# JanEGerken/HEAL-SWIN

Hardware: AMD Instinct MI355X
Metric: images/sec fwd+bwd, HEAL-SWIN nside=256 seg, batch=8 at 1/2/4/8 MI355X (higher is better)
Workload: dtype bf16

## Files before the change

heal_swin_amd/_lib.py:

```python
import ctypes
import os

import numpy as np

_PKG = os.path.dirname(os.path.abspath(__file__))
LIB_PATH = os.path.join(_PKG, "lib", "libhealswin.so")

HS_F32, HS_BF16 = 0, 1
HS_F64 = 3
HS_PRED_LABELS, HS_PRED_ROWS16 = 2, 4
HS_ENSEMBLE_PROB, HS_ENSEMBLE_LOGIT = 0, 1
HS_ATTN_COSINE = 1
HS_ATTN_FORCE_VALU = 2
HS_ATTN_RESIDUAL = 4
HS_ATTN_OVERWRITE_GRADS = 8
HS_EPI_BIAS, HS_EPI_GELU, HS_EPI_DGELU, HS_EPI_RESID = 0, 1, 2, 3
HS_ACC_DEFER = 2
HS_MLP_NORM_AFTER = 16
HS_U8, HS_I32, HS_I64 = 8, 9, 10
HS_FLAT_PATCH_ROWS, HS_FLAT_PIXEL_ROWS, HS_FLAT_IMAGE = 0, 1, 2
HS_DEPTH_L1, HS_DEPTH_L2, HS_DEPTH_HUBER, HS_DEPTH_LOGVAR = 0, 1, 2, 3
HS_DT_NONE, HS_DT_LOG, HS_DT_INV = 0, 1, 2
HS_DT_ZERO_BKG, HS_DT_1000_BKG, HS_DT_AFFINE, HS_DT_INVERSE = 1, 2, 4, 8
HS_DEPTH_STATS_WORDS = 15
# ... 157 lines not shown
    "hs_grad_scale": [c_ptr, c_i64, c_float, c_ptr, c_ptr],
    "hs_weight_avg_update": [c_ptr, c_ptr, c_i64, c_int, c_float, c_ptr, c_ptr, c_int, c_ptr],
    "hs_weight_avg_advance": [c_ptr, c_ptr, c_int, c_ptr],
    "hs_weight_avg_swap": [c_ptr, c_ptr, c_ptr, c_i64, c_ptr],
    "hs_split_bf16x3": [c_ptr, c_ptr, c_i64, c_int, c_int, c_ptr],
    "hs_gelu_split3": [c_ptr, c_ptr, c_ptr, c_i64, c_int, ctypes.c_float, ctypes.c_uint64, c_ptr],
    "hs_linear_wgrad_ld": [c_ptr, c_i64, c_i64, c_ptr, c_i64, c_i64, c_ptr, c_ptr, c_ptr, c_i64, c_int, c_int, c_int, c_ptr],
    "hs_layernorm_fwd": [c_ptr, c_ptr, c_ptr, c_ptr, c_ptr, c_ptr, c_ptr, c_i64, c_int, c_int, c_ptr],
    "hs_add_layernorm_fwd": [c_ptr, c_ptr, c_ptr, c_ptr, c_ptr, c_ptr, c_ptr, c_ptr, c_i64, c_int, c_int, c_ptr],
    "hs_add_layernorm_bwd": [c_ptr, c_ptr, c_ptr, c_ptr, c_ptr, c_ptr, c_ptr, c_ptr, c_ptr, c_ptr, c_int, c_i64, c_int, c_int, c_ptr],
    "hs_layernorm_drop_fwd": [c_ptr, c_ptr, c_ptr, c_ptr, c_ptr, c_ptr, c_ptr, c_ptr, c_i64, ctypes.c_float, ctypes.c_uint64,
                              c_i64, c_int, c_int, c_ptr],
    "hs_layernorm_drop_bwd": [c_ptr, c_ptr, c_ptr, c_ptr, c_ptr, c_ptr, c_ptr, c_ptr, c_ptr, c_int, c_ptr, c_i64, ctypes.c_float,
                              ctypes.c_uint64, c_i64, c_int, c_int, c_ptr],
    "hs_add_layernorm_drop_fwd": [c_ptr, c_ptr, c_ptr, c_ptr, c_ptr, c_ptr, c_ptr, c_ptr, c_ptr, c_i64, ctypes.c_float,
                                  ctypes.c_uint64, c_i64, c_int, c_int, c_ptr],
    "hs_layernorm_fwd_ex": [c_ptr, c_ptr, c_ptr, c_ptr, c_ptr, c_ptr, c_ptr, c_ptr, c_ptr, c_ptr, c_ptr, c_ptr, c_i64, ctypes.c_float,
                            ctypes.c_uint64, c_i64, c_int, c_int, c_ptr],
    "hs_add_layernorm_drop_bwd": [c_ptr, c_ptr, c_ptr, c_ptr, c_ptr, c_ptr, c_ptr, c_ptr, c_ptr, c_ptr, c_ptr, c_int, c_ptr, c_i64,
                                  ctypes.c_float, ctypes.c_uint64, c_i64, c_int, c_int, c_ptr],
    "hs_seg_ce_fwd": [c_ptr, c_ptr, c_ptr, c_ptr, c_i64, c_i64, c_int, c_i64, c_i64, c_i64, c_int, c_i64, c_int, c_ptr],
    "hs_seg_ce_bwd": [c_ptr, c_ptr, c_ptr, c_ptr, c_ptr, c_i64, c_i64, c_int, c_i64, c_i64, c_i64, c_i64, c_i64, c_i64, c_int, c_i64,
                      c_int, c_ptr],
    "hs_depth_loss_fwd": [c_ptr, c_ptr, c_ptr, c_i64, c_i64, c_int, c_i64, c_i64, c_i64, c_int, c_float, c_int, c_ptr],
    "hs_depth_loss_bwd": [c_ptr, c_ptr, c_ptr, c_ptr, c_i64, c_i64, c_int, c_i64, c_i64, c_i64, c_i64, c_i64, c_i64, c_int, c_float, c_int, c_ptr],
    "hs_gemm_nt": [c_ptr, c_i64, c_ptr, c_i64, c_int, c_ptr, c_i64, c_ptr, c_i64, c_int, c_ptr, c_ptr, c_ptr, c_i64, c_int, c_int,
                   ctypes.c_float, ctypes.c_uint64, c_int, c_ptr],
    "hs_lib_gemm_supported": [],
    "hs_lib_gemm_set_supported": [c_int],
    "hs_lib_gemm_nt": [c_ptr, c_ptr, c_ptr, c_int, c_ptr, c_ptr, c_i64, c_int, c_int, c_ptr],
    "hs_lib_gemm_pick": [c_i64, c_int, c_int, c_int, ctypes.POINTER(c_int), ctypes.POINTER(c_int), ctypes.c_char_p, c_int],
    "hs_lib_gemm_set_pick": [c_i64, c_int, c_int, c_int, c_int],
    "hs_gemm_nt_set_tile": [c_int],
    "hs_gemm_nt_tile_variant": [c_i64, c_int, c_int, c_int, c_int],
    "hs_set_reserved_cus": [c_int],
    "hs_transpose_many_16": [c_ptr, c_int, c_int, c_ptr],
    "hs_debug_occupy_cus": [c_int, c_int, c_int, ctypes.c_double, c_ptr],
    "hs_debug_buffer_soffset_probe": [c_ptr, c_int, c_int, c_ptr, c_ptr],
    "hs_window_attn_module_supported": [c_int, c_int, c_int, c_int],
    "hs_window_attn_module_fwd": [c_ptr, c_ptr, c_ptr, c_ptr, c_ptr, c_ptr, c_ptr, c_ptr, c_ptr, c_ptr, c_ptr, c_i64, c_ptr, c_int, c_i64,
                                  c_int, c_int, c_int, c_uint, c_int, c_ptr],
    "hs_window_attn_module_fwd_train": [c_ptr] * 17 + [c_i64] + [c_ptr] * 6 + [c_int, c_i64, c_int, c_int, c_int, c_uint, c_int, c_ptr],
    "hs_window_attn_module_bwd_chain": [c_ptr] * 14 + [c_i64] + [c_ptr] * 11 + [c_int, c_int, c_i64, c_int, c_int, c_int, c_uint, c_int, c_ptr],
    "hs_layernorm_bwd": [c_ptr, c_ptr, c_ptr, c_ptr, c_ptr, c_ptr, c_ptr, c_ptr, c_ptr, c_int, c_i64, c_int, c_int, c_ptr],
    "hs_patch_merge_fwd": [c_ptr, c_ptr, c_ptr, c_ptr, c_ptr, c_ptr, c_ptr, c_ptr, c_i64, c_int, c_int, c_int, c_ptr],
    "hs_patch_merge_bwd": [c_ptr, c_ptr, c_ptr, c_ptr, c_ptr, c_ptr, c_ptr, c_ptr, c_ptr, c_ptr, c_ptr, c_ptr, c_ptr, c_int, c_i64,
                           c_int, c_int, c_int, c_ptr],
    "hs_patch_expand_fwd": [c_ptr, c_ptr, c_ptr, c_ptr, c_ptr, c_ptr, c_ptr, c_ptr, c_i64, c_int, c_int, c_int, c_int, c_ptr],
    "hs_patch_expand_bwd": [c_ptr, c_ptr, c_ptr, c_ptr, c_ptr, c_ptr, c_ptr, c_ptr, c_ptr, c_ptr, c_ptr, c_ptr, c_ptr, c_int, c_i64,
                            c_int, c_int, c_int, c_int, c_ptr],
}
_OTHER = {
    "hs_version": ([], ctypes.c_char_p),
    "hs_last_error": ([], ctypes.c_char_p),
    "hs_status_string": ([c_int], ctypes.c_char_p),
    "hs_device_count": ([], c_int),
    "hs_get_reserved_cus": ([], c_int),
    "hs_grad_guard_piece": ([], c_int),
    "hs_adam_max_groups": ([], c_int),
    "hs_get_seed_epoch": ([], c_ptr),
    "hs_reduce_pending": ([c_ptr], c_int),
    "hs_layernorm_bwd_workspace": ([c_i64, c_int], c_i64),
    "hs_seg_ce_partials": ([c_i64, c_i64], c_i64),
    "hs_depth_loss_partials": ([c_i64, c_i64], c_i64),
    "hs_depth_points_workspace": ([c_i64, c_i64], c_i64),
    "hs_depth_metrics_partials": ([c_i64], c_i64),
# ... 163 lines not shown
```

heal_swin_amd/csrc/expand_ln_head.hip:

```cpp
#include "ln_head_device.h"
#include "hs_depth_loss.h"

#pragma clang fp contract(off)
#include "hs_depth_target.h"
#include "hs_depth_metrics.h"
#pragma clang fp contract(fast)

namespace hs {
namespace {

constexpr int kP = 4;
constexpr int kRowB = 256;
constexpr int kPatchRow = 128;

constexpr int kHistBins = kKP * kKP;

__device__ __forceinline__ int argmax_merge(float best, int arg, float ob, int oa) {
    const bool n0 = best != best, n1 = ob != ob;
    const int lower = arg < oa ? arg : oa;
    if (n0 || n1) return n0 && n1 ? lower : (n0 ? arg : oa);
    return best > ob ? arg : (ob > best ? oa : lower);
}

struct TailLane {
    float num = 0.f, den = 0.f;
    uint32_t pred4 = 0;
    uint32_t bad_rows = 0;
    uint32_t* hist = nullptr;
    float4 m4, lv4;
    double dsum[depth_metrics::kNSums];
};

struct TailCe {
    const uint8_t* labels;
    const float* class_w;
    float* loss_part;
    int n_classes;
    __device__ __forceinline__ bool has_loss() const { return labels != nullptr; }
    __device__ __forceinline__ bool ce_row(TailLane& st, const f32x16& lg, const float (&bk)[8], int64_t orow, bool live, int half,
                                           float (&v)[8], int& yl) const {
        if (!labels) return false;
        float m = -INFINITY;
#pragma unroll
        for (int r = 0; r < 8; ++r) {
            v[r] = lg[r] + bk[r];
            if (class_natural(r, half) < n_classes) m = fmaxf(m, v[r]);
        }
        m = fmaxf(m, __shfl_xor(m, 32, 64));
        yl = live ? (int)labels[orow] : 255;
        float ssum = 0.f, pick = 0.f;
#pragma unroll
        for (int r = 0; r < 8; ++r) {
            const int cls = class_natural(r, half);
            if (cls < n_classes) ssum += __builtin_amdgcn_exp2f((v[r] - m) * kLog2e);
            pick = cls == yl ? v[r] : pick;
        }
        ssum += __shfl_xor(ssum, 32, 64);
        pick += __shfl_xor(pick, 32, 64);
        const float wy = yl < n_classes ? (class_w ? class_w[yl] : 1.f) : 0.f;
        if (half == 0) {
            st.num = fmaf(wy, m + __builtin_amdgcn_logf(ssum) * kLn2 - pick, st.num);
            st.den += wy;
        }
        return true;
    }
    __device__ __forceinline__ void row(TailLane& st, const f32x16& lg, const float (&bk)[8], int64_t orow, int, bool live,
                                        int lane) const {
        float v[8];
        int yl;
        ce_row(st, lg, bk, orow, live, lane >> 5, v, yl);
    }
};

struct TailCeStep : TailCe {
    uint8_t* preds;
    unsigned long long* conf;
    unsigned long long* bad;
    __device__ __forceinline__ bool has_loss() const { return true; }
    __device__ __forceinline__ void row(TailLane& st, const f32x16& lg, const float (&bk)[8], int64_t orow, int p, bool live,
                                        int lane) const {
        const int half = lane >> 5;
        float v[8];
        int yl;
        if (!ce_row(st, lg, bk, orow, live, half, v, yl)) return;
        float best = -INFINITY;
        int arg = 4 * half < n_classes ? 4 * half : 64;
#pragma unroll
        for (int r = 0; r < 8; ++r) {
            const int cls = class_natural(r, half);
            if (cls < n_classes && !(best != best) && (v[r] > best || v[r] != v[r])) {
                best = v[r];
                arg = cls;
            }
        }
        const int pred = argmax_merge(best, arg, __shfl_xor(best, 32, 64), __shfl_xor(arg, 32, 64));
        st.pred4 |= (uint32_t)pred << (8 * p);
        if (conf) {
            const bool mine = live && half == 0;
            const int bin = mine && yl < n_classes ? yl * n_classes + pred : -1;
            st.bad_rows += (uint32_t)__popcll(__ballot(mine && yl >= n_classes));
            const int lead = __builtin_amdgcn_readfirstlane(bin);
            const unsigned long long same = __ballot(bin == lead);
            if (bin == lead) {
                if (lead >= 0 && lane == __ffsll((long long)same) - 1) atomicAdd(&st.hist[lead], (uint32_t)__popcll(same));
            } else if (bin >= 0) {
                atomicAdd(&st.hist[bin], 1u);
            }
        }
    }
};

struct TailDepth {
    const float* target;
    float* loss_part;
    int kind;
    float delta;
    __device__ __forceinline__ bool has_loss() const { return true; }
    __device__ __forceinline__ float depth_row(TailLane& st, const f32x16& lg, const float (&bk)[8], int64_t orow, bool live,
                                               int half) const {
        const float t = live && half == 0 ? target[orow] : INFINITY;
        if (depth_keep(t)) {
            st.num += depth_term(kind, delta, lg[0] + bk[0], lg[1] + bk[1], t);
            st.den += 1.f;
        }
        return t;
    }
    __device__ __forceinline__ void row(TailLane& st, const f32x16& lg, const float (&bk)[8], int64_t orow, int, bool live,
                                        int lane) const {
        depth_row(st, lg, bk, orow, live, lane >> 5);
    }
};

struct TailDepthStep : TailDepth {
    int n_out;
    TargetOp inv;
    depth_metrics::Rule rule;
    double* partial;
    float* preds;
    float* logvar_out;
    int64_t rows;
    __device__ __forceinline__ void row(TailLane& st, const f32x16& lg, const float (&bk)[8], int64_t orow, int p, bool live,
                                        int lane) const {
        const int half = lane >> 5;
        const float p0 = lg[0] + bk[0], p1 = lg[1] + bk[1], t = depth_row(st, lg, bk, orow, live, half);
        if (partial || preds) {
#pragma clang fp contract(off)
            const float m = target_op(p0, inv);
            if (partial && live && half == 0)
                depth_metrics::accumulate<float, float>(st.dsum, rule, m, target_op(t, inv), [&] { return p1; });
            st.m4.x = p == 0 ? m : st.m4.x;
            st.m4.y = p == 1 ? m : st.m4.y;
            st.m4.z = p == 2 ? m : st.m4.z;
            st.m4.w = p == 3 ? m : st.m4.w;
        }
        st.lv4.x = p == 0 ? p1 : st.lv4.x;
        st.lv4.y = p == 1 ? p1 : st.lv4.y;
        st.lv4.z = p == 2 ? p1 : st.lv4.z;
        st.lv4.w = p == 3 ? p1 : st.lv4.w;
    }
};

template <int NB, typename Loss>
__global__ void __launch_bounds__(256, 1) expand_ln_head_fwd_kernel(const uint16_t* __restrict__ xn, const uint16_t* __restrict__ xn_lo,
                                                                    const uint16_t* __restrict__ wexp,
                                                                    const uint16_t* __restrict__ wfold, const float* __restrict__ bvec,
                                                                    uint16_t* __restrict__ y, float* __restrict__ logits,
                                                                    float* __restrict__ mean_out, float* __restrict__ rstd_out,
                                                                    int64_t tokens, Loss ce) {
    constexpr bool kStep = std::is_same<Loss, TailCeStep>::value, kDStep = std::is_same<Loss, TailDepthStep>::value;
    constexpr int C = 32 * NB, KS = 2 * NB, NCH = C / 8;
    extern __shared__ __attribute__((aligned(16))) unsigned char smem[];
    unsigned char* wl = smem;
    unsigned char* patch = smem + kP * C * kRowB + (threadIdx.x >> 6) * (32 * kPatchRow);
    const int tid = threadIdx.x, lane = tid & 63, l31 = lane & 31, half = lane >> 5;

    for (int q = tid; q < kP * C * NCH; q += 256) {
        const int row = q / NCH, ch = q % NCH;
        *(uint4*)(wl + row * kRowB + ((ch ^ (row & 15)) << 4)) = *(const uint4*)(wexp + (int64_t)row * C + ch * 8);
    }
    bf16x8 wfa[NB][2], wfl[NB][2];
#pragma unroll
    for (int ct = 0; ct < NB; ++ct)
#pragma unroll
        for (int j = 0; j < 2; ++j) {
            const uint16_t* src = wfold + l31 * C + 32 * ct + 16 * j + 4 * half;
            const uint2 a = *(const uint2*)src, b = *(const uint2*)(src + 8);
            wfa[ct][j] = __builtin_bit_cast(bf16x8, make_uint4(a.x, a.y, b.x, b.y));
            const uint2 al = *(const uint2*)(src + 32 * C), bl = *(const uint2*)(src + 32 * C + 8);
            wfl[ct][j] = __builtin_bit_cast(bf16x8, make_uint4(al.x, al.y, bl.x, bl.y));
        }
    float bk[8];
    load_head_bias(bvec, half, bk);
    uint32_t* hist = (uint32_t*)(smem + kP * C * kRowB + 4 * 32 * kPatchRow);
    TailLane st;
    st.hist = hist + (tid >> 6) * kHistBins;
    if constexpr (kStep) {
        for (int j = tid; j < 4 * kHistBins; j += 256) hist[j] = 0;
    }
    if constexpr (kDStep) {
#pragma unroll
        for (int k = 0; k < depth_metrics::kNSums; ++k) st.dsum[k] = 0.0;
    }
    __syncthreads();

    const int sx = l31 & 15;
    const int64_t wave = (int64_t)blockIdx.x * 4 + (tid >> 6), nwaves = (int64_t)gridDim.x * 4;
    for (int64_t tok0 = wave * 32; tok0 < tokens; tok0 += nwaves * 32) {
        const int64_t tok = tok0 + l31;
        const bool live = tok < tokens;
        bf16x8 xb[KS];
#pragma unroll
        for (int ks = 0; ks < KS; ++ks) {
            const uint4 v = live ? *(const uint4*)(xn + tok * C + 16 * ks + 8 * half) : make_uint4(0, 0, 0, 0);
            xb[ks] = __builtin_bit_cast(bf16x8, v);
        }
        st.pred4 = 0;
        st.m4 = st.lv4 = make_float4(0.f, 0.f, 0.f, 0.f);
#pragma unroll 1
        for (int p = 0; p < kP; ++p) {
            f32x16 acc[NB];
#pragma unroll
            for (int ct = 0; ct < NB; ++ct)
#pragma unroll
                for (int r = 0; r < 16; ++r) acc[ct][r] = 0.f;
            const unsigned char* wrow = wl + (p * C + l31) * kRowB;
#pragma unroll
            for (int ks = 0; ks < KS; ++ks) {
                const int co = ((2 * ks + half) ^ sx) << 4;
#pragma unroll
                for (int ct = 0; ct < NB; ++ct) {
                    const bf16x8 a = *(const bf16x8*)(wrow + ct * 32 * kRowB + co);
                    acc[ct] = __builtin_amdgcn_mfma_f32_32x32x16_bf16(a, xb[ks], acc[ct], 0, 0, 0);
                }
            }
            if (xn_lo) {
#pragma unroll
                for (int ks = 0; ks < KS; ++ks) {
                    const uint4 v = live ? *(const uint4*)(xn_lo + tok * C + 16 * ks + 8 * half) : make_uint4(0, 0, 0, 0);
                    const int co = ((2 * ks + half) ^ sx) << 4;
#pragma unroll
                    for (int ct = 0; ct < NB; ++ct) {
                        const bf16x8 a = *(const bf16x8*)(wrow + ct * 32 * kRowB + co);
                        acc[ct] = __builtin_amdgcn_mfma_f32_32x32x16_bf16(a, __builtin_bit_cast(bf16x8, v), acc[ct], 0, 0, 0);
                    }
                }
            }
            const int64_t orow = tok * kP + p;
            if (y) {
#pragma unroll
                for (int pr = 0; pr < (NB + 1) / 2; ++pr) {
#pragma unroll
                    for (int t = 0; t < 2; ++t) {
                        const int ct = 2 * pr + t;
                        if (ct < NB) {
#pragma unroll
                            for (int g = 0; g < 4; ++g) {
                                const int chunk = 4 * t + g;
                                *(uint2*)(patch + l31 * kPatchRow + ((chunk ^ (l31 & 7)) << 4) + 8 * half) =
                                    make_uint2(pack_bf16x2(acc[ct][4 * g], acc[ct][4 * g + 1]), pack_bf16x2(acc[ct][4 * g + 2], acc[ct][4 * g + 3]));
                            }
                        }
                    }
                    __builtin_amdgcn_fence(__ATOMIC_RELEASE, "wavefront");
                    __builtin_amdgcn_wave_barrier();
                    constexpr int kChunksLast = (NB % 2) ? 4 : 8;
                    const int nchunks = (2 * pr + 1 < NB) ? 8 : kChunksLast;
#pragma unroll
                    for (int i = 0; i < 4; ++i) {
                        const int q = lane + 64 * i, row = q >> 3, chunk = q & 7;
                        const uint4 v = *(const uint4*)(patch + row * kPatchRow + ((chunk ^ (row & 7)) << 4));
                        if (chunk < nchunks && tok0 + row < tokens)
                            *(uint4*)(y + ((tok0 + row) * kP + p) * C + 64 * pr + chunk * 8) = v;
                    }
                    __builtin_amdgcn_fence(__ATOMIC_ACQUIRE, "wavefront");
                    __builtin_amdgcn_wave_barrier();
                }
            }
            float mean, rstd;
            row_stats<16>(acc, mean, rstd);
            f32x16 lg;
#pragma unroll
            for (int r = 0; r < 16; ++r) lg[r] = 0.f;
#pragma unroll
            for (int ct = 0; ct < NB; ++ct)
#pragma unroll
                for (int j = 0; j < 2; ++j) {
                    float xh[8];
#pragma unroll
                    for (int i = 0; i < 8; ++i) xh[i] = acc[ct][8 * j + i] * rstd;
                    lg = head_step<3>(lg, xh, wfa[ct][j], wfl[ct][j]);
                }
            ce.row(st, lg, bk, orow, p, live, lane);
            if (live) {
                if (logits) {
                    *(float4*)(logits + orow * kKP + 4 * half) = make_float4(lg[0] + bk[0], lg[1] + bk[1], lg[2] + bk[2], lg[3] + bk[3]);
                    *(float4*)(logits + orow * kKP + 8 + 4 * half) = make_float4(lg[4] + bk[4], lg[5] + bk[5], lg[6] + bk[6], lg[7] + bk[7]);
                }
                if (half == 0 && mean_out) {
                    mean_out[orow] = mean;
                    rstd_out[orow] = rstd;
                }
            }
        }
        if constexpr (kStep) {
            if (ce.preds && live && half == 0) *(uint32_t*)(ce.preds + tok * kP) = st.pred4;
        }
        if constexpr (kDStep) {
            if (live && half == 0) {
                if (ce.preds) *(float4*)(ce.preds + tok * kP) = st.m4;
                float* lv = ce.preds ? (ce.n_out > 1 ? ce.preds + ce.rows : nullptr) : ce.logvar_out;
                if (lv) *(float4*)(lv + tok * kP) = st.lv4;
            }
        }
    }
    if constexpr (kDStep) {
        if (ce.partial) {
            constexpr int NS = depth_metrics::kNSums;
            static_assert(NS * 256 * sizeof(double) <= kP * 64 * kRowB + 4 * 32 * kPatchRow, "lane sums must fit the LDS at C = 64");
            double* red = (double*)smem;
            __syncthreads();
#pragma unroll
            for (int k = 0; k < NS; ++k) red[k * 256 + tid] = st.dsum[k];
            __syncthreads();
            for (int h = 128; h > 0; h >>= 1) {
                for (int q = tid; q < NS * h; q += 256) {
                    const int k = q / h, j = q - k * h;
                    red[k * 256 + j] += red[k * 256 + j + h];
                }
                __syncthreads();
            }
            if (tid < NS) ce.partial[(int64_t)blockIdx.x * NS + tid] = red[tid * 256];
        }
    }
    if constexpr (kStep) {
        if (ce.conf) {
            __syncthreads();
            const int bins = ce.n_classes * ce.n_classes;
            if (tid < bins) {
                const uint32_t n = hist[tid] + hist[kHistBins + tid] + hist[2 * kHistBins + tid] + hist[3 * kHistBins + tid];
                if (n) atomicAdd(&ce.conf[tid], (unsigned long long)n);
            }
            if (lane == 0 && st.bad_rows) atomicAdd(&ce.bad[0], (unsigned long long)st.bad_rows);
        }
    }
    if (ce.has_loss()) {
        const float n = wave_sum(st.num), d = wave_sum(st.den);
        if (lane == 0) {
            ce.loss_part[2 * wave] = n;
            ce.loss_part[2 * wave + 1] = d;
        }
    }
}

}
}

extern "C" {

int hs_expand_ln_head_supported(int width, int children, int n_classes, int dtype) {
    return dtype == HS_BF16 && children == hs::kP && width % 32 == 0 && width >= 64 && width <= 128 && n_classes >= 1 && n_classes <= 16;
}

extern "C++" {
namespace {
template <typename Loss>
int launch_expand_ln_head(const void* xn, const void* xn_lo, const void* wexp, const void* wfold, const float* bvec, void* y, float* logits,
                          float* mean, float* rstd, int64_t tokens, int width, int children, int dtype, void* stream, Loss ce,
                          const char* who) {
    using namespace hs;
    HS_CHECK_ARG(xn && wexp && wfold && bvec, "%s: null pointer", who);
    HS_CHECK_ARG(tokens > 0, "%s: bad shape", who);
    HS_CHECK_ARG((y == nullptr) == (mean == nullptr) && (mean == nullptr) == (rstd == nullptr),
                 "%s: y, mean and rstd (what the backward needs) go together", who);
    if (!hs_expand_ln_head_supported(width, children, 1, dtype))
        return fail(HS_ERR_UNSUPPORTED, "%s: bf16, 4 children, C in {64, 96, 128} (got C = %d, children %d): the expand "
                    "weight must fit the LDS", who, width, children);
    HS_CHECK_ALIGNED(who, 16, xn, xn_lo, wexp, wfold, bvec, y);
    constexpr bool kStep = std::is_same<Loss, TailCeStep>::value;
    const size_t smem = (size_t)kP * width * kRowB + 4 * 32 * kPatchRow + (kStep ? 4 * kHistBins * sizeof(uint32_t) : 0);
    HS_CHECK_ARG(smem <= 160 * 1024, "%s: %zu bytes of LDS", who, smem);
    const dim3 grid((unsigned)hs_expand_ln_head_blocks(tokens)), block(256);
    if constexpr (kStep) {
        const int64_t groups = (tokens + 31) / 32, waves = (int64_t)grid.x * 4;
        HS_CHECK_ARG((groups + waves - 1) / waves < (1ll << 25), "%s: %lld tokens on %lld waves overflow the 32-bit histogram bins", who,
                     (long long)tokens, (long long)waves);
    }
    return with_width_blocks<4>(width, [&](auto nb) {
        auto kern = expand_ln_head_fwd_kernel<decltype(nb)::value, Loss>;
        static bool configured = false;
        if (!configured) {
            HS_HIP_CHECK(hipFuncSetAttribute((const void*)kern, hipFuncAttributeMaxDynamicSharedMemorySize, (int)smem));
            configured = true;
        }
        hipLaunchKernelGGL(kern, grid, block, smem, (hipStream_t)stream, (const uint16_t*)xn, (const uint16_t*)xn_lo,
                           (const uint16_t*)wexp, (const uint16_t*)wfold, bvec, (uint16_t*)y, logits, mean, rstd, tokens, ce);
        HS_LAUNCH_CHECK("expand_ln_head_fwd");
        return (int)HS_OK;
    });
}
int check_ce_loss(const char* who, const void* labels, const void* loss_partials, int n_classes) {
    HS_CHECK_ARG(labels && loss_partials, "%s: null pointer", who);
    return hs::check_class_count(who, n_classes);
}
int check_depth_loss(const char* who, const void* target, const void* loss_partials, int kind, float huber_delta, int n_out) {
    HS_CHECK_ARG(target && loss_partials, "%s: null pointer", who);
    return hs::check_depth_head(who, kind, huber_delta, n_out);
}
}
}

int64_t hs_expand_ln_head_blocks(int64_t tokens) {
    int64_t blocks = (tokens + 127) / 128;
    const int cus = hs::usable_cus();
    if (blocks > cus) blocks = cus;
    return blocks < 1 ? 1 : blocks;
}

int hs_expand_ln_head_fwd(const void* xn, const void* xn_lo, const void* wexp, const void* wfold, const float* bvec, void* y, float* logits,
                          float* mean, float* rstd, int64_t tokens, int width, int children, int dtype, void* stream) {
    HS_CHECK_ARG(logits, "hs_expand_ln_head_fwd: null pointer");
    return launch_expand_ln_head(xn, xn_lo, wexp, wfold, bvec, y, logits, mean, rstd, tokens, width, children, dtype, stream,
                                 hs::TailCe{nullptr, nullptr, nullptr, 0}, "hs_expand_ln_head_fwd");
}

int hs_expand_ln_head_ce_fwd(const void* xn, const void* xn_lo, const void* wexp, const void* wfold, const float* bvec, const uint8_t* labels,
                             const float* class_weights, int n_classes, void* y, float* logits, float* mean, float* rstd,
                             float* loss_partials, int64_t tokens, int width, int children, int dtype, void* stream) {
    if (int e = check_ce_loss("hs_expand_ln_head_ce_fwd", labels, loss_partials, n_classes)) return e;
    return launch_expand_ln_head(xn, xn_lo, wexp, wfold, bvec, y, logits, mean, rstd, tokens, width, children, dtype, stream,
                                 hs::TailCe{labels, class_weights, loss_partials, n_classes}, "hs_expand_ln_head_ce_fwd");
}

int hs_expand_ln_head_ce_step_fwd(const void* xn, const void* xn_lo, const void* wexp, const void* wfold, const float* bvec,
                                  const uint8_t* labels, const float* class_weights, int n_classes, void* y, float* logits, float* mean,
                                  float* rstd, float* loss_partials, uint8_t* preds, int64_t* confmat, int64_t* bad, int64_t tokens,
                                  int width, int children, int dtype, void* stream) {
    const char* who = "hs_expand_ln_head_ce_step_fwd";
    if (int e = check_ce_loss(who, labels, loss_partials, n_classes)) return e;
    HS_CHECK_ARG(!confmat || bad, "%s: confmat needs bad (the counter of labels >= n_classes)", who);
    HS_CHECK_ARG(((uintptr_t)preds & 3) == 0, "%s: preds must be 4-byte aligned", who);
    return launch_expand_ln_head(xn, xn_lo, wexp, wfold, bvec, y, logits, mean, rstd, tokens, width, children, dtype, stream,
                                 hs::TailCeStep{{labels, class_weights, loss_partials, n_classes}, preds, (unsigned long long*)confmat,
                                                (unsigned long long*)bad}, who);
}

int hs_expand_ln_head_depth_step_fwd(const void* xn, const void* xn_lo, const void* wexp, const void* wfold, const float* bvec,
                                     const float* target, int kind, float huber_delta, int n_out, void* y, float* logits, float* mean,
                                     float* rstd, float* loss_partials, int flags, int transform, float shift, float scale, int use_logvar,
                                     double total_mean, const float* ranges, int n_ranges, double* metric_partials, double* metric_state,
                                     float* preds, float* logvar_out, int64_t tokens, int width, int children, int dtype, void* stream) {
    const char* who = "hs_expand_ln_head_depth_step_fwd";
    if (int e = check_depth_loss(who, target, loss_partials, kind, huber_delta, n_out)) return e;
    HS_CHECK_ARG(transform == HS_DT_NONE || transform == HS_DT_LOG || transform == HS_DT_INV, "%s: transform %d", who, transform);
    HS_CHECK_ARG((flags & ~(HS_DT_AFFINE | HS_DT_INVERSE)) == 0, "%s: flags %d (HS_DT_AFFINE or 0: the inverse chain is applied)", who, flags);
    HS_CHECK_ARG((metric_partials == nullptr) == (metric_state == nullptr), "%s: metric_partials and metric_state go together", who);
    HS_CHECK_ARG(n_out == 2 || !(logvar_out || (use_logvar && metric_state)), "%s: the log variance needs a two-channel head", who);
    hs::TailDepthStep st{{target, loss_partials, kind, huber_delta}, n_out, hs::TargetOp{flags | HS_DT_INVERSE, transform, shift, scale},
                         {}, metric_partials, preds, logvar_out, tokens * hs::kP};
    if (int e = hs::depth_metrics::fill_rule(st.rule, use_logvar, total_mean, ranges, n_ranges)) return e;
    HS_CHECK_ALIGNED(who, 16, preds, logvar_out);
    HS_CHECK_ALIGNED(who, 8, metric_partials, metric_state);
    HS_CHECK_ALIGNED(who, 4, target, loss_partials);
    if (int e = launch_expand_ln_head(xn, xn_lo, wexp, wfold, bvec, y, logits, mean, rstd, tokens, width, children, dtype, stream, st, who))
        return e;
    if (metric_state) {
        hipLaunchKernelGGL(hs::depth_metrics::reduce_kernel, dim3(1), dim3(hs::depth_metrics::kThreads), 0, (hipStream_t)stream,
                           metric_partials, (int)hs_expand_ln_head_blocks(tokens), metric_state);
        HS_LAUNCH_CHECK("expand_ln_head_depth_step_reduce");
    }
    return HS_OK;
}

int hs_expand_ln_head_depth_fwd(const void* xn, const void* xn_lo, const void* wexp, const void* wfold, const float* bvec, const float* target,
                                int kind, float huber_delta, int n_out, void* y, float* logits, float* mean, float* rstd, float* loss_partials,
                                int64_t tokens, int width, int children, int dtype, void* stream) {
    if (int e = check_depth_loss("hs_expand_ln_head_depth_fwd", target, loss_partials, kind, huber_delta, n_out)) return e;
    return launch_expand_ln_head(xn, xn_lo, wexp, wfold, bvec, y, logits, mean, rstd, tokens, width, children, dtype, stream,
                                 hs::TailDepth{target, loss_partials, kind, huber_delta}, "hs_expand_ln_head_depth_fwd");
}

}
```

include/healswin.h:

```cpp
#ifndef HEALSWIN_H
#define HEALSWIN_H

#include <stdint.h>

#ifdef __cplusplus
extern "C" {
#endif

typedef enum {
    HS_OK = 0,
    HS_ERR_INVALID_ARG = 1,
    HS_ERR_UNSUPPORTED = 2,
    HS_ERR_HIP = 3,
    HS_ERR_NOT_PERMUTATION = 4,
    HS_ERR_MISALIGNED = 5
} hs_status;

typedef enum { HS_F32 = 0, HS_BF16 = 1 } hs_dtype;

#define HS_ATTN_COSINE 1u
#define HS_ATTN_FORCE_VALU 2u
#define HS_ATTN_RESIDUAL 4u
#define HS_ATTN_OVERWRITE_GRADS 8u

// ... 364 lines not shown
int hs_sample_bilinear_u8_f32_per_sample(const void* img, int batch, int channels, int height, int width, const double* rx,
                                         const double* ry, int64_t n, float* out, void* stream);
int hs_sample_nearest_f32_per_sample(const float* src, int batch, int height, int width, const double* rx, const double* ry, int64_t n,
                                     float background, float* out, void* stream);
int hs_depth_target(const float* in, int64_t in_stride_b, int64_t in_stride_p, float* out, int64_t out_stride_b, int64_t out_stride_p,
                    int64_t batch, int64_t n, int flags, int transform, float shift, float scale, void* stream);
int64_t hs_depth_stats_partials(int64_t n);
int hs_depth_stats_update(const float* depth, int64_t n, int transform, int use_masking, int64_t* partial, int64_t* state, void* stream);
int hs_depth_stats_merge(const int64_t* states, int count, int64_t* state, void* stream);
int hs_histogram_update(const float* depth, int64_t n, int transform, int use_masking, const double* edges, int bins, int64_t* counts,
                        void* stream);

int64_t hs_select_rows_workspace(int rows);
int hs_select_rows(const float* x, int rows, int64_t n, int64_t row_stride, int64_t k, int nan_propagates, int splits, void* workspace,
                   float* out, void* stream);

int hs_ln_head_supported(int width, int n_classes, int dtype);
int64_t hs_ln_head_partials(int64_t rows);
int hs_ln_head_fwd(const void* y, const void* wfold, const float* bvec, void* logits, float* mean, float* rstd, int64_t rows,
                   int width, int dtype, int logits_dtype, void* stream);
int hs_ln_head_bwd(const void* y, const float* mean, const float* rstd, const void* dlogits, const void* afold, void* dy,
                   void* dprime, float* partials, int64_t rows, int width, int dtype, int logits_dtype, void* stream);

int hs_split_bf16x3(const float* x, void* out, int64_t rows, int k, int mode, void* stream);
int hs_gelu_split3(const float* dy, const float* x, void* out3, int64_t rows, int k, float drop_p, uint64_t seed, void* stream);
int hs_linear_wgrad_ld(const void* dy, int64_t ldy, int64_t ycol0, const void* x, int64_t ldx, int64_t xcol0, float* dw, float* dbias,
                       float* workspace, int64_t rows, int n_out, int k_in, int accumulate, void* stream);

int hs_expand_ln_head_supported(int width, int children, int n_classes, int dtype);
int hs_expand_ln_head_fwd(const void* xn, const void* xn_lo, const void* wexp, const void* wfold, const float* bvec, void* y, float* logits,
                          float* mean, float* rstd, int64_t tokens, int width, int children, int dtype, void* stream);

int64_t hs_expand_ln_head_blocks(int64_t tokens);
int hs_expand_ln_head_ce_fwd(const void* xn, const void* xn_lo, const void* wexp, const void* wfold, const float* bvec, const uint8_t* labels,
                             const float* class_weights, int n_classes, void* y, float* logits, float* mean, float* rstd,
                             float* loss_partials, int64_t tokens, int width, int children, int dtype, void* stream);
int hs_expand_ln_head_ce_step_fwd(const void* xn, const void* xn_lo, const void* wexp, const void* wfold, const float* bvec,
                                  const uint8_t* labels, const float* class_weights, int n_classes, void* y, float* logits, float* mean,
                                  float* rstd, float* loss_partials, uint8_t* preds, int64_t* confmat, int64_t* bad, int64_t tokens,
                                  int width, int children, int dtype, void* stream);
int hs_ln_head_ce_bwd(const void* y, const float* mean, const float* rstd, const uint8_t* labels, const float* class_weights,
                      const float* scale, int n_classes, const void* wfold, const float* bvec, const void* afold, void* dy, void* dprime,
                      float* partials, int64_t rows, int width, int dtype, void* stream);

int hs_expand_ln_head_depth_fwd(const void* xn, const void* xn_lo, const void* wexp, const void* wfold, const float* bvec, const float* target,
                                int kind, float huber_delta, int n_out, void* y, float* logits, float* mean, float* rstd, float* loss_partials,
                                int64_t tokens, int width, int children, int dtype, void* stream);
int hs_expand_ln_head_depth_step_fwd(const void* xn, const void* xn_lo, const void* wexp, const void* wfold, const float* bvec,
                                     const float* target, int kind, float huber_delta, int n_out, void* y, float* logits, float* mean,
                                     float* rstd, float* loss_partials, int flags, int transform, float shift, float scale, int use_logvar,
                                     double total_mean, const float* ranges, int n_ranges, double* metric_partials, double* metric_state,
                                     float* preds, float* logvar_out, int64_t tokens, int width, int children, int dtype, void* stream);
int hs_ln_head_depth_bwd(const void* y, const float* mean, const float* rstd, const float* target, int kind, float huber_delta,
                         const float* scale, int n_out, const void* wfold, const float* bvec, const void* afold, void* dy, void* dprime,
                         float* partials, int64_t rows, int width, int dtype, void* stream);

int hs_patch_merge_fwd(const void* x, const float* gamma, const float* beta, const void* w, void* normed, float* mean, float* rstd,
                       void* out, int64_t rows, int dim, int dim_out, int dtype, void* stream);
int64_t hs_patch_merge_bwd_workspace(int64_t rows, int dim, int dim_out);
int hs_patch_merge_bwd(const void* dout, const void* x, const void* normed, const float* gamma, const float* mean, const float* rstd,
                       const void* w_t, void* dnormed, void* dx, float* dw, float* dgamma, float* dbeta, float* workspace,
                       int accumulate, int64_t rows, int dim, int dim_out, int dtype, void* stream);
int hs_patch_expand_fwd(const void* x, const void* w, const float* gamma, const float* beta, void* expanded, float* mean, float* rstd,
                        void* out, int64_t rows, int dim, int dim_exp, int children, int dtype, void* stream);
int64_t hs_patch_expand_bwd_workspace(int64_t rows, int dim, int dim_exp, int children);
int hs_patch_expand_bwd(const void* dout, const void* x, const void* expanded, const float* gamma, const float* mean, const float* rstd,
// ... 30 lines not shown
```

Measured before the change: 57.23.

## Run expand-LN-head tail kernel with 8 waves per block and lean register use

Adds an 8-wave-per-workgroup variant of the fused expand+layernorm+head kernel, the default for CE losses. To fit registers it reloads the input per child instead of holding it across the loop, shrinks the patch staging buffer for the step variant, and prefetches four labels per token with class weights shuffled across lanes instead of loaded per row. Loss partials from the extra waves are folded through LDS so the partial-buffer layout stays 4 slots per block, and unused slots are zeroed. The aim is more latency hiding per CU, paid for with extra global reloads and tighter LDS use.

```diff
diff --git a/heal_swin_amd/_lib.py b/heal_swin_amd/_lib.py
--- a/heal_swin_amd/_lib.py
+++ b/heal_swin_amd/_lib.py
@@ -213,6 +213,9 @@
     "hs_lib_gemm_pick": [c_i64, c_int, c_int, c_int, ctypes.POINTER(c_int), ctypes.POINTER(c_int), ctypes.c_char_p, c_int],
     "hs_lib_gemm_set_pick": [c_i64, c_int, c_int, c_int, c_int],
     "hs_gemm_nt_set_tile": [c_int],
+    "hs_expand_ln_head_set_waves": [c_int],
+    "hs_expand_ln_head_set_max_blocks": [c_int],
+    "hs_expand_ln_head_waves": [c_int],
     "hs_gemm_nt_tile_variant": [c_i64, c_int, c_int, c_int, c_int],
     "hs_set_reserved_cus": [c_int],
     "hs_transpose_many_16": [c_ptr, c_int, c_int, c_ptr],
diff --git a/heal_swin_amd/csrc/expand_ln_head.hip b/heal_swin_amd/csrc/expand_ln_head.hip
--- a/heal_swin_amd/csrc/expand_ln_head.hip
+++ b/heal_swin_amd/csrc/expand_ln_head.hip
@@ -27,6 +27,8 @@
     uint32_t pred4 = 0;
     uint32_t bad_rows = 0;
     uint32_t* hist = nullptr;
+    uint32_t lab4 = 0;
+    float cw = 1.f;
     float4 m4, lv4;
     double dsum[depth_metrics::kNSums];
 };
@@ -37,7 +39,19 @@
     float* loss_part;
     int n_classes;
     __device__ __forceinline__ bool has_loss() const { return labels != nullptr; }
-    __device__ __forceinline__ bool ce_row(TailLane& st, const f32x16& lg, const float (&bk)[8], int64_t orow, bool live, int half,
+    __device__ __forceinline__ void prepare(TailLane& st, int lane) const {
+        if (labels) st.cw = class_w ? ((lane & 15) < n_classes ? class_w[lane & 15] : 0.f) : 1.f;
+    }
+    __device__ __forceinline__ void fetch(TailLane& st, int64_t tok, bool live) const {
+        if (!labels) return;
+        const uint8_t* lp = labels + tok * 4;
+        if (((uintptr_t)labels & 3) == 0)
+            st.lab4 = live ? *(const uint32_t*)lp : 0xffffffffu;
+        else
+            st.lab4 = live ? (uint32_t)lp[0] | (uint32_t)lp[1] << 8 | (uint32_t)lp[2] << 16 | (uint32_t)lp[3] << 24 : 0xffffffffu;
+    }
+    template <bool PRE>
+    __device__ __forceinline__ bool ce_row(TailLane& st, const f32x16& lg, const float (&bk)[8], int64_t orow, int p, bool live, int half,
                                            float (&v)[8], int& yl) const {
         if (!labels) return false;
         float m = -INFINITY;
@@ -47,7 +61,7 @@
             if (class_natural(r, half) < n_classes) m = fmaxf(m, v[r]);
         }
         m = fmaxf(m, __shfl_xor(m, 32, 64));
-        yl = live ? (int)labels[orow] : 255;
+        yl = PRE ? (int)((st.lab4 >> (8 * p)) & 255u) : (live ? (int)labels[orow] : 255);
         float ssum = 0.f, pick = 0.f;
 #pragma unroll
         for (int r = 0; r < 8; ++r) {
@@ -57,18 +71,25 @@
         }
         ssum += __shfl_xor(ssum, 32, 64);
         pick += __shfl_xor(pick, 32, 64);
-        const float wy = yl < n_classes ? (class_w ? class_w[yl] : 1.f) : 0.f;
+        float wy;
+        if constexpr (PRE) {
+            const float wsh = __shfl(st.cw, yl & 15, 64);
+            wy = yl < n_classes ? wsh : 0.f;
+        } else {
+            wy = yl < n_classes ? (class_w ? class_w[yl] : 1.f) : 0.f;
+        }
         if (half == 0) {
             st.num = fmaf(wy, m + __builtin_amdgcn_logf(ssum) * kLn2 - pick, st.num);
             st.den += wy;
         }
         return true;
     }
-    __device__ __forceinline__ void row(TailLane& st, const f32x16& lg, const float (&bk)[8], int64_t orow, int, bool live,
+    template <bool PRE>
+    __device__ __forceinline__ void row(TailLane& st, const f32x16& lg, const float (&bk)[8], int64_t orow, int p, bool live,
                                         int lane) const {
         float v[8];
         int yl;
-        ce_row(st, lg, bk, orow, live, lane >> 5, v, yl);
+        ce_row<PRE>(st, lg, bk, orow, p, live, lane >> 5, v, yl);
     }
 };
 
@@ -77,12 +98,13 @@
     unsigned long long* conf;
     unsigned long long* bad;
     __device__ __forceinline__ bool has_loss() const { return true; }
+    template <bool PRE>
     __device__ __forceinline__ void row(TailLane& st, const f32x16& lg, const float (&bk)[8], int64_t orow, int p, bool live,
                                         int lane) const {
         const int half = lane >> 5;
         float v[8];
         int yl;
-        if (!ce_row(st, lg, bk, orow, live, half, v, yl)) return;
+        if (!ce_row<PRE>(st, lg, bk, orow, p, live, half, v, yl)) return;
         float best = -INFINITY;
         int arg = 4 * half < n_classes ? 4 * half : 64;
 #pragma unroll
@@ -125,6 +147,9 @@
         }
         return t;
     }
+    __device__ __forceinline__ void prepare(TailLane&, int) const {}
+    __device__ __forceinline__ void fetch(TailLane&, int64_t, bool) const {}
+    template <bool>
     __device__ __forceinline__ void row(TailLane& st, const f32x16& lg, const float (&bk)[8], int64_t orow, int, bool live,
                                         int lane) const {
         depth_row(st, lg, bk, orow, live, lane >> 5);
@@ -139,6 +164,7 @@
     float* preds;
     float* logvar_out;
     int64_t rows;
+    template <bool>
     __device__ __forceinline__ void row(TailLane& st, const f32x16& lg, const float (&bk)[8], int64_t orow, int p, bool live,
                                         int lane) const {
         const int half = lane >> 5;
@@ -160,21 +186,34 @@
     }
 };
 
-template <int NB, typename Loss>
-__global__ void __launch_bounds__(256, 1) expand_ln_head_fwd_kernel(const uint16_t* __restrict__ xn, const uint16_t* __restrict__ xn_lo,
-                                                                    const uint16_t* __restrict__ wexp,
-                                                                    const uint16_t* __restrict__ wfold, const float* __restrict__ bvec,
-                                                                    uint16_t* __restrict__ y, float* __restrict__ logits,
-                                                                    float* __restrict__ mean_out, float* __restrict__ rstd_out,
-                                                                    int64_t tokens, Loss ce) {
+template <int NB, int NW, typename Loss>
+constexpr int patch_rows() {
+    return NB == 4 && NW == 8 && std::is_same<Loss, TailCeStep>::value ? 16 : 32;
+}
+template <int NB, int NW, typename Loss>
+constexpr size_t tail_smem() {
+    return (size_t)kP * 32 * NB * kRowB + NW * patch_rows<NB, NW, Loss>() * kPatchRow +
+           (std::is_same<Loss, TailCeStep>::value ? NW * kHistBins * sizeof(uint32_t) : 0);
+}
+
+template <int NB, int NW, typename Loss>
+__global__ void __launch_bounds__(64 * NW, 1) expand_ln_head_fwd_kernel(const uint16_t* __restrict__ xn, const uint16_t* __restrict__ xn_lo,
+                                                                        const uint16_t* __restrict__ wexp,
+                                                                        const uint16_t* __restrict__ wfold, const float* __restrict__ bvec,
+                                                                        uint16_t* __restrict__ y, float* __restrict__ logits,
+                                                                        float* __restrict__ mean_out, float* __restrict__ rstd_out,
+                                                                        int64_t tokens, int64_t n_parts, Loss ce) {
     constexpr bool kStep = std::is_same<Loss, TailCeStep>::value, kDStep = std::is_same<Loss, TailDepthStep>::value;
     constexpr int C = 32 * NB, KS = 2 * NB, NCH = C / 8;
+    constexpr int NT = 64 * NW, PR = patch_rows<NB, NW, Loss>();
+    constexpr bool kLean = NW == 8;
+    static_assert(!kDStep || NW == 4, "the lane-sum tree of TailDepthStep is laid out for 256 lanes");
     extern __shared__ __attribute__((aligned(16))) unsigned char smem[];
     unsigned char* wl = smem;
-    unsigned char* patch = smem + kP * C * kRowB + (threadIdx.x >> 6) * (32 * kPatchRow);
+    unsigned char* patch = smem + kP * C * kRowB + (threadIdx.x >> 6) * (PR * kPatchRow);
     const int tid = threadIdx.x, lane = tid & 63, l31 = lane & 31, half = lane >> 5;
 
-    for (int q = tid; q < kP * C * NCH; q += 256) {
+    for (int q = tid; q < kP * C * NCH; q += NT) {
         const int row = q / NCH, ch = q % NCH;
         *(uint4*)(wl + row * kRowB + ((ch ^ (row & 15)) << 4)) = *(const uint4*)(wexp + (int64_t)row * C + ch * 8);
     }
@@ -189,13 +228,15 @@
             const uint2 al = *(const uint2*)(src + 32 * C), bl = *(const uint2*)(src + 32 * C + 8);
             wfl[ct][j] = __builtin_bit_cast(bf16x8, make_uint4(al.x, al.y, bl.x, bl.y));
         }
+    constexpr bool kLeanBias = kLean && kStep && NB == 4;
     float bk[8];
-    load_head_bias(bvec, half, bk);
-    uint32_t* hist = (uint32_t*)(smem + kP * C * kRowB + 4 * 32 * kPatchRow);
+    if constexpr (!kLeanBias) load_head_bias(bvec, half, bk);
+    uint32_t* hist = (uint32_t*)(smem + kP * C * kRowB + NW * PR * kPatchRow);
     TailLane st;
     st.hist = hist + (tid >> 6) * kHistBins;
+    if constexpr (kLean) ce.prepare(st, lane);
     if constexpr (kStep) {
-        for (int j = tid; j < 4 * kHistBins; j += 256) hist[j] = 0;
+        for (int j = tid; j < NW * kHistBins; j += NT) hist[j] = 0;
     }
     if constexpr (kDStep) {
 #pragma unroll
@@ -204,16 +245,19 @@
     __syncthreads();
 
     const int sx = l31 & 15;
-    const int64_t wave = (int64_t)blockIdx.x * 4 + (tid >> 6), nwaves = (int64_t)gridDim.x * 4;
+    const int64_t wave = (int64_t)blockIdx.x * NW + (tid >> 6), nwaves = (int64_t)gridDim.x * NW;
     for (int64_t tok0 = wave * 32; tok0 < tokens; tok0 += nwaves * 32) {
         const int64_t tok = tok0 + l31;
         const bool live = tok < tokens;
         bf16x8 xb[KS];
-#pragma unroll
-        for (int ks = 0; ks < KS; ++ks) {
-            const uint4 v = live ? *(const uint4*)(xn + tok * C + 16 * ks + 8 * half) : make_uint4(0, 0, 0, 0);
-            xb[ks] = __builtin_bit_cast(bf16x8, v);
-        }
+        if constexpr (!kLean) {
+#pragma unroll
+            for (int ks = 0; ks < KS; ++ks) {
+                const uint4 v = live ? *(const uint4*)(xn + tok * C + 16 * ks + 8 * half) : make_uint4(0, 0, 0, 0);
+                xb[ks] = __builtin_bit_cast(bf16x8, v);
+            }
+        }
+        if constexpr (kLean) ce.fetch(st, tok, live);
         st.pred4 = 0;
         st.m4 = st.lv4 = make_float4(0.f, 0.f, 0.f, 0.f);
 #pragma unroll 1
@@ -224,6 +268,15 @@
 #pragma unroll
                 for (int r = 0; r < 16; ++r) acc[ct][r] = 0.f;
             const unsigned char* wrow = wl + (p * C + l31) * kRowB;
+            if constexpr (kLean) {
+                int64_t xoff = tok * C + 8 * half;
+                asm volatile("" : "+v"(xoff));
+#pragma unroll
+                for (int ks = 0; ks < KS; ++ks) {
+                    const uint4 v = live ? *(const uint4*)(xn + xoff + 16 * ks) : make_uint4(0, 0, 0, 0);
+                    xb[ks] = __builtin_bit_cast(bf16x8, v);
+                }
+            }
 #pragma unroll
             for (int ks = 0; ks < KS; ++ks) {
                 const int co = ((2 * ks + half) ^ sx) << 4;
@@ -234,13 +287,16 @@
                 }
             }
             if (xn_lo) {
+                int woff = (p * C + l31) * kRowB;
+                if constexpr (kLean) asm volatile("" : "+v"(woff));
+                const unsigned char* wrow2 = wl + woff;
 #pragma unroll
                 for (int ks = 0; ks < KS; ++ks) {
                     const uint4 v = live ? *(const uint4*)(xn_lo + tok * C + 16 * ks + 8 * half) : make_uint4(0, 0, 0, 0);
                     const int co = ((2 * ks + half) ^ sx) << 4;
 #pragma unroll
                     for (int ct = 0; ct < NB; ++ct) {
-                        const bf16x8 a = *(const bf16x8*)(wrow + ct * 32 * kRowB + co);
+                        const bf16x8 a = *(const bf16x8*)(wrow2 + ct * 32 * kRowB + co);
                         acc[ct] = __builtin_amdgcn_mfma_f32_32x32x16_bf16(a, __builtin_bit_cast(bf16x8, v), acc[ct], 0, 0, 0);
                     }
                 }
@@ -250,30 +306,36 @@
 #pragma unroll
                 for (int pr = 0; pr < (NB + 1) / 2; ++pr) {
 #pragma unroll
-                    for (int t = 0; t < 2; ++t) {
-                        const int ct = 2 * pr + t;
-                        if (ct < NB) {
-#pragma unroll
-                            for (int g = 0; g < 4; ++g) {
-                                const int chunk = 4 * t + g;
-                                *(uint2*)(patch + l31 * kPatchRow + ((chunk ^ (l31 & 7)) << 4) + 8 * half) =
-                                    make_uint2(pack_bf16x2(acc[ct][4 * g], acc[ct][4 * g + 1]), pack_bf16x2(acc[ct][4 * g + 2], acc[ct][4 * g + 3]));
+                    for (int rb = 0; rb < 32; rb += PR) {
+                        if (PR == 32 || (l31 & PR) == rb) {
+#pragma unroll
+                            for (int t = 0; t < 2; ++t) {
+                                const int ct = 2 * pr + t;
+                                if (ct < NB) {
+#pragma unroll
+                                    for (int g = 0; g < 4; ++g) {
+                                        const int chunk = 4 * t + g;
+                                        *(uint2*)(patch + (l31 & (PR - 1)) * kPatchRow + ((chunk ^ (l31 & 7)) << 4) + 8 * half) =
+                                            make_uint2(pack_bf16x2(acc[ct][4 * g], acc[ct][4 * g + 1]),
+                                                       pack_bf16x2(acc[ct][4 * g + 2], acc[ct][4 * g + 3]));
+                                    }
+                                }
                             }
                         }
+                        __builtin_amdgcn_fence(__ATOMIC_RELEASE, "wavefront");
+                        __builtin_amdgcn_wave_barrier();
+                        constexpr int kChunksLast = (NB % 2) ? 4 : 8;
+                        const int nchunks = (2 * pr + 1 < NB) ? 8 : kChunksLast;
+#pragma unroll
+                        for (int i = 0; i < PR / 8; ++i) {
+                            const int q = lane + 64 * i, prow = q >> 3, row = rb + prow, chunk = q & 7;
+                            const uint4 v = *(const uint4*)(patch + prow * kPatchRow + ((chunk ^ (prow & 7)) << 4));
+                            if (chunk < nchunks && tok0 + row < tokens)
+                                *(uint4*)(y + ((tok0 + row) * kP + p) * C + 64 * pr + chunk * 8) = v;
+                        }
+                        __builtin_amdgcn_fence(__ATOMIC_ACQUIRE, "wavefront");
+                        __builtin_amdgcn_wave_barrier();
                     }
-                    __builtin_amdgcn_fence(__ATOMIC_RELEASE, "wavefront");
-                    __builtin_amdgcn_wave_barrier();
-                    constexpr int kChunksLast = (NB % 2) ? 4 : 8;
-                    const int nchunks = (2 * pr + 1 < NB) ? 8 : kChunksLast;
-#pragma unroll
-                    for (int i = 0; i < 4; ++i) {
-                        const int q = lane + 64 * i, row = q >> 3, chunk = q & 7;
-                        const uint4 v = *(const uint4*)(patch + row * kPatchRow + ((chunk ^ (row & 7)) << 4));
-                        if (chunk < nchunks && tok0 + row < tokens)
-                            *(uint4*)(y + ((tok0 + row) * kP + p) * C + 64 * pr + chunk * 8) = v;
-                    }
-                    __builtin_amdgcn_fence(__ATOMIC_ACQUIRE, "wavefront");
-                    __builtin_amdgcn_wave_barrier();
                 }
             }
             float mean, rstd;
@@ -290,7 +352,12 @@
                     for (int i = 0; i < 8; ++i) xh[i] = acc[ct][8 * j + i] * rstd;
                     lg = head_step<3>(lg, xh, wfa[ct][j], wfl[ct][j]);
                 }
-            ce.row(st, lg, bk, orow, p, live, lane);
+            if constexpr (kLeanBias) {
+                int h = half;
+                asm volatile("" : "+v"(h));
+                load_head_bias(bvec, h, bk);
+            }
+            ce.template row<kLean>(st, lg, bk, orow, p, live, lane);
             if (live) {
                 if (logits) {
                     *(float4*)(logits + orow * kKP + 4 * half) = make_float4(lg[0] + bk[0], lg[1] + bk[1], lg[2] + bk[2], lg[3] + bk[3]);
@@ -337,17 +404,32 @@
             __syncthreads();
             const int bins = ce.n_classes * ce.n_classes;
             if (tid < bins) {
-                const uint32_t n = hist[tid] + hist[kHistBins + tid] + hist[2 * kHistBins + tid] + hist[3 * kHistBins + tid];
+                uint32_t n = 0;
+#pragma unroll
+                for (int w = 0; w < NW; ++w) n += hist[w * kHistBins + tid];
                 if (n) atomicAdd(&ce.conf[tid], (unsigned long long)n);
             }
             if (lane == 0 && st.bad_rows) atomicAdd(&ce.bad[0], (unsigned long long)st.bad_rows);
         }
     }
     if (ce.has_loss()) {
-        const float n = wave_sum(st.num), d = wave_sum(st.den);
-        if (lane == 0) {
-            ce.loss_part[2 * wave] = n;
-            ce.loss_part[2 * wave + 1] = d;
+        float n = wave_sum(st.num), d = wave_sum(st.den);
+        const int w = tid >> 6;
+        if constexpr (NW == 8) {
+            float2* ex = (float2*)(smem + kP * C * kRowB);
+            __syncthreads();
+            if (w >= 4 && lane == 0) ex[w - 4] = make_float2(n, d);
+            __syncthreads();
+            if (w < 4 && lane == 0) {
+                n += ex[w].x;
+                d += ex[w].y;
+            }
+        }
+        if (w < 4 && lane == 0) {
+            const int64_t slot = (int64_t)blockIdx.x * 4 + w, slots = (int64_t)gridDim.x * 4;
+            ce.loss_part[2 * slot] = n;
+            ce.loss_part[2 * slot + 1] = d;
+            for (int64_t j = slot + slots; j < n_parts; j += slots) ce.loss_part[2 * j] = ce.loss_part[2 * j + 1] = 0.f;
         }
     }
 }
@@ -363,6 +445,49 @@
 
 extern "C++" {
 namespace {
+int g_tail_waves = getenv("HS_TAIL_WAVES") ? atoi(getenv("HS_TAIL_WAVES")) : 0;
+
+template <typename Loss>
+int tail_waves() {
+    constexpr bool kDepth = std::is_base_of<hs::TailDepth, Loss>::value;
+    return kDepth || g_tail_waves == 4 ? 4 : 8;
+}
+
+int g_tail_max_blocks = 0;
+
+int tail_cus() {
+    const int cus = hs::usable_cus();
+    return g_tail_max_blocks > 0 && g_tail_max_blocks < cus ? g_tail_max_blocks : cus;
+}
+int64_t tail_grid(int64_t tokens, int waves) {
+    const int64_t per = 32 * (int64_t)waves, blocks = (tokens + per - 1) / per;
+    return blocks < 1 ? 1 : (blocks > tail_cus() ? tail_cus() : blocks);
+}
+
+template <int NB, int NW, typename Loss>
+int launch_tail_variant(const void* xn, const void* xn_lo, const void* wexp, const void* wfold, const float* bvec, void* y, float* logits,
+                        float* mean, float* rstd, int64_t tokens, void* stream, Loss ce, const char* who) {
+    using namespace hs;
+    constexpr size_t smem = tail_smem<NB, NW, Loss>();
+    static_assert(smem <= 160 * 1024, "the workgroup's LDS");
+    const dim3 grid((unsigned)tail_grid(tokens, NW)), block(64 * NW);
+    if constexpr (std::is_same<Loss, TailCeStep>::value) {
+        const int64_t groups = (tokens + 31) / 32, waves = (int64_t)grid.x * NW;
+        HS_CHECK_ARG((groups + waves - 1) / waves < (1ll << 25), "%s: %lld tokens on %lld waves overflow the 32-bit histogram bins", who,
+                     (long long)tokens, (long long)waves);
+    }
+    auto kern = expand_ln_head_fwd_kernel<NB, NW, Loss>;
+    static bool configured = false;
+    if (!configured) {
+        HS_HIP_CHECK(hipFuncSetAttribute((const void*)kern, hipFuncAttributeMaxDynamicSharedMemorySize, (int)smem));
+        configured = true;
+    }
+    hipLaunchKernelGGL(kern, grid, block, smem, (hipStream_t)stream, (const uint16_t*)xn, (const uint16_t*)xn_lo, (const uint16_t*)wexp,
+                       (const uint16_t*)wfold, bvec, (uint16_t*)y, logits, mean, rstd, tokens, 4 * hs_expand_ln_head_blocks(tokens), ce);
+    HS_LAUNCH_CHECK("expand_ln_head_fwd");
+    return (int)HS_OK;
+}
+
 template <typename Loss>
 int launch_expand_ln_head(const void* xn, const void* xn_lo, const void* wexp, const void* wfold, const float* bvec, void* y, float* logits,
                           float* mean, float* rstd, int64_t tokens, int width, int children, int dtype, void* stream, Loss ce,
@@ -376,26 +501,13 @@
         return fail(HS_ERR_UNSUPPORTED, "%s: bf16, 4 children, C in {64, 96, 128} (got C = %d, children %d): the expand "
                     "weight must fit the LDS", who, width, children);
     HS_CHECK_ALIGNED(who, 16, xn, xn_lo, wexp, wfold, bvec, y);
-    constexpr bool kStep = std::is_same<Loss, TailCeStep>::value;
-    const size_t smem = (size_t)kP * width * kRowB + 4 * 32 * kPatchRow + (kStep ? 4 * kHistBins * sizeof(uint32_t) : 0);
-    HS_CHECK_ARG(smem <= 160 * 1024, "%s: %zu bytes of LDS", who, smem);
-    const dim3 grid((unsigned)hs_expand_ln_head_blocks(tokens)), block(256);
-    if constexpr (kStep) {
-        const int64_t groups = (tokens + 31) / 32, waves = (int64_t)grid.x * 4;
-        HS_CHECK_ARG((groups + waves - 1) / waves < (1ll << 25), "%s: %lld tokens on %lld waves overflow the 32-bit histogram bins", who,
-                     (long long)tokens, (long long)waves);
-    }
+    const bool wide = tail_waves<Loss>() == 8;
     return with_width_blocks<4>(width, [&](auto nb) {
-        auto kern = expand_ln_head_fwd_kernel<decltype(nb)::value, Loss>;
-        static bool configured = false;
-        if (!configured) {
-            HS_HIP_CHECK(hipFuncSetAttribute((const void*)kern, hipFuncAttributeMaxDynamicSharedMemorySize, (int)smem));
-            configured = true;
-        }
-        hipLaunchKernelGGL(kern, grid, block, smem, (hipStream_t)stream, (const uint16_t*)xn, (const uint16_t*)xn_lo,
-                           (const uint16_t*)wexp, (const uint16_t*)wfold, bvec, (uint16_t*)y, logits, mean, rstd, tokens, ce);
-        HS_LAUNCH_CHECK("expand_ln_head_fwd");
-        return (int)HS_OK;
+        constexpr int NB = decltype(nb)::value;
+        if constexpr (!std::is_base_of<TailDepth, Loss>::value) {
+            if (wide) return launch_tail_variant<NB, 8>(xn, xn_lo, wexp, wfold, bvec, y, logits, mean, rstd, tokens, stream, ce, who);
+        }
+        return launch_tail_variant<NB, 4>(xn, xn_lo, wexp, wfold, bvec, y, logits, mean, rstd, tokens, stream, ce, who);
     });
 }
 int check_ce_loss(const char* who, const void* labels, const void* loss_partials, int n_classes) {
@@ -409,12 +521,20 @@
 }
 }
 
-int64_t hs_expand_ln_head_blocks(int64_t tokens) {
-    int64_t blocks = (tokens + 127) / 128;
-    const int cus = hs::usable_cus();
-    if (blocks > cus) blocks = cus;
-    return blocks < 1 ? 1 : blocks;
-}
+int64_t hs_expand_ln_head_blocks(int64_t tokens) { return tail_grid(tokens, 4); }
+
+int hs_expand_ln_head_set_waves(int waves) {
+    g_tail_waves = waves;
+    return HS_OK;
+}
+
+int hs_expand_ln_head_set_max_blocks(int max_blocks) {
+    HS_CHECK_ARG(max_blocks >= 0, "hs_expand_ln_head_set_max_blocks: %d", max_blocks);
+    g_tail_max_blocks = max_blocks;
+    return HS_OK;
+}
+
+int hs_expand_ln_head_waves(int depth_loss) { return depth_loss ? tail_waves<hs::TailDepth>() : tail_waves<hs::TailCe>(); }
 
 int hs_expand_ln_head_fwd(const void* xn, const void* xn_lo, const void* wexp, const void* wfold, const float* bvec, void* y, float* logits,
                           float* mean, float* rstd, int64_t tokens, int width, int children, int dtype, void* stream) {
@@ -465,7 +585,7 @@
         return e;
     if (metric_state) {
         hipLaunchKernelGGL(hs::depth_metrics::reduce_kernel, dim3(1), dim3(hs::depth_metrics::kThreads), 0, (hipStream_t)stream,
-                           metric_partials, (int)hs_expand_ln_head_blocks(tokens), metric_state);
+                           metric_partials, (int)tail_grid(tokens, tail_waves<hs::TailDepthStep>()), metric_state);
         HS_LAUNCH_CHECK("expand_ln_head_depth_step_reduce");
     }
     return HS_OK;
diff --git a/include/healswin.h b/include/healswin.h
--- a/include/healswin.h
+++ b/include/healswin.h
@@ -420,6 +420,9 @@
                           float* mean, float* rstd, int64_t tokens, int width, int children, int dtype, void* stream);
 
 int64_t hs_expand_ln_head_blocks(int64_t tokens);
+int hs_expand_ln_head_set_waves(int waves);
+int hs_expand_ln_head_set_max_blocks(int max_blocks);
+int hs_expand_ln_head_waves(int depth_loss);
 int hs_expand_ln_head_ce_fwd(const void* xn, const void* xn_lo, const void* wexp, const void* wfold, const float* bvec, const uint8_t* labels,
                              const float* class_weights, int n_classes, void* y, float* logits, float* mean, float* rstd,
                              float* loss_partials, int64_t tokens, int width, int children, int dtype, void* stream);
```

New measurement: 57.33, median of 6. Within noise of the previous version (+0.2%).
